# lgen-sudo/EgoM2P

Measured on AMD Instinct MI355X. Metric: multimodal tokens/sec (ego-b 400M, 10300-tok clips), training fwd+bwd+allreduce+AdamW, higher is better.
Workload: dtype bf16; 1 GPU; egom2p_base_12e_12d_swiglu_nobias mod4, synthetic 10300-position clips (1009+1009 rgb, 1009+1009 depth, 15+15 cam, 15+15 gaze kept -> N=M=2048), bf16 MFMA GEMM/attention, fp32 residual/LN/CE/AdamW; micro_batch=64, global_batch=256, parallelism=dp1

## Files before the change

egom2p_amd/_lib.py:

```python
from __future__ import annotations

import ctypes as C
import os

_HERE = os.path.dirname(os.path.abspath(__file__))
LIB_PATH = os.environ.get("EGOM2P_HIP_LIB", os.path.join(_HERE, "libegom2p_hip.so"))
MAX_MODS = 8

ABI_VERSION = 12
EPI_BF16, EPI_F32, EPI_RESID, EPI_BIAS_RESID, EPI_BIAS_BF16 = 0, 1, 2, 3, 4

vp, i32, i64, f32 = C.c_void_p, C.c_int, C.c_long, C.c_float


class CompactDesc(C.Structure):
    _fields_ = [
        ("n_mods", i32), ("n_keep", i32), ("is_decoder", i32),
        ("mask", vp * MAX_MODS), ("ids", vp * MAX_MODS), ("dam", vp * MAX_MODS),
        ("n_pos", i32 * MAX_MODS), ("mod_id", i32 * MAX_MODS),
        ("ids_keep", vp), ("pad", vp), ("mod_mask", vp), ("slot", vp), ("local", vp), ("tok", vp),
        ("ks", vp), ("ke", vp), ("n_valid", vp), ("seg", vp), ("err", vp), ("seg_bad", vp), ("n_reg", i32),
    ]


# ... 120 lines not shown
    "ego_cast_weight": [vp, i32, i32, i64, vp, i64, vp, i64, i32, vp],
    "ego_cast_f32_bf16": [vp, vp, i64, vp],
    "ego_bias_grad_work_floats": [i64, i32],
    "ego_bias_grad": [vp, i64, i32, vp, vp, i64, vp],
    "ego_grad_sqnorm": [vp, i64, vp, vp, vp],
    "ego_adamw_step": [vp, vp, vp, vp, i64, f32, f32, f32, f32, f32, i32, f32, f32, vp, i32, vp],
    "ego_adamw_gate": [vp, f32, f32, i32, vp, vp],
    "ego_adamw_step_gated": [vp, vp, vp, vp, i64, f32, f32, f32, f32, f32, i32, f32, f32, vp, i32, vp, vp],
    "ego_ema_update": [vp, vp, i64, f32, f32, vp],
    "ego_swap_f32": [vp, vp, i64, vp],
    "ego_sample_cfg_topp": [vp, vp, i64, i32, f32, f32, i32, f32, vp, vp, vp, i32, vp],
    "ego_maskgit_positions": [vp, i32, i32, i32, vp, vp],
    "ego_maskgit_select": [vp, vp, vp, i32, i32, i32, i32, vp, vp, vp, vp, vp],
    "ego_dp_unique_id": [vp],
    "ego_dp_comm_create": [vp, i32, i32, C.POINTER(vp)],
    "ego_dp_comm_destroy": [vp],
    "ego_dp_allreduce_begin": [vp, vp, i64, i32, vp, vp],
    "ego_dp_wait": [vp, vp, vp],
}

EXPORTS = tuple(_SIGS)

_SIGS_OPTIM = {
    "ego_adamw_step_seg": [vp, vp, vp, vp, i64, C.POINTER(AdamwSeg), vp, i32, vp, C.POINTER(AdamwHp), f32, f32, f32, f32, f32, vp, i32,
                           vp, vp],
}
EXPORTS_OPTIM = tuple(_SIGS_OPTIM)

OPT_ADAM, OPT_SGD, OPT_NESTEROV = 1, 2, 3
_SIGS_OPTIM_KINDS = {
    "ego_optim_step_seg": _SIGS_OPTIM["ego_adamw_step_seg"][:-1] + [i32, f32, vp],
}
EXPORTS_OPTIM_KINDS = tuple(_SIGS_OPTIM_KINDS)
_lib = None


class EgoHipError(RuntimeError):
    pass


def load():
    global _lib
    if _lib is None:
        if not os.path.exists(LIB_PATH):
            raise EgoHipError(
                f"{LIB_PATH} not found: build it with `python -c 'import __graft_entry__ as g; g.build()'` "
                "(or `make -C egom2p_amd/csrc`). There is no CPU fallback for the product path.")
        import torch
        hip_rt = os.path.join(os.path.dirname(torch.__file__), "lib", "libamdhip64.so")
        if os.path.exists(hip_rt):
            C.CDLL(hip_rt, mode=C.RTLD_GLOBAL)
        lib = C.CDLL(LIB_PATH)
        for name, args in {**_SIGS, **_SIGS_OPTIM, **_SIGS_OPTIM_KINDS}.items():
            fn = getattr(lib, name)
            fn.argtypes = args
            fn.restype = i64 if name.endswith(("_work_floats", "_split_floats", "_work_ints")) else i32
        if lib.ego_abi_version() != ABI_VERSION:
            raise EgoHipError(f"libegom2p_hip.so ABI version {lib.ego_abi_version()} != binding {ABI_VERSION}: rebuild (make -C egom2p_amd/csrc)")
        if "EGO_GEMM_NT256" in os.environ or "EGO_GEMM_TN256" in os.environ:
            lib.ego_gemm_kernel_mode(int(os.environ.get("EGO_GEMM_NT256", "1")), int(os.environ.get("EGO_GEMM_TN256", "1")))
        if "EGO_GEMM_SMALL_TILES" in os.environ:
            lib.ego_gemm_small_tiles(int(os.environ["EGO_GEMM_SMALL_TILES"]))
        _lib = lib
    return _lib


def check(rc: int, what: str):
    if rc != 0:
        raise EgoHipError(f"{what} failed: {'bad arguments' if rc == 1 else 'kernel launch failed'} (rc={rc})")
```

egom2p_amd/csrc/rowops.hip:

```cpp
#include "common.h"
#include "egom2p_hip.h"

namespace {

__device__ __forceinline__ float mul_then_add(float a, float b, float c) {
#pragma clang fp contract(off)
    const float t = a * b;
    return t + c;
}
__device__ __forceinline__ float mul_rounded(float a, float b) {
#pragma clang fp contract(off)
    return a * b;
}

constexpr int LN_MAXC_MAX = 8;

template <int LN_MAXC, bool TAIL, bool BIAS = false>
__global__ __launch_bounds__(256) void ln_fwd_kernel(const float* __restrict__ x, const float* __restrict__ w,
                                                     bf16_t* __restrict__ y, float* __restrict__ mean_out,
                                                     float* __restrict__ rstd_out, const int* __restrict__ out_row,
                                                     int rows, int D, int ld, float eps, unsigned char* __restrict__ q8, long ldq,
                                                     float* __restrict__ qscale, const float* __restrict__ b = nullptr) {
#pragma clang fp contract(off)
    const int lane = threadIdx.x & 63;
    const int row = blockIdx.x * 4 + __builtin_amdgcn_readfirstlane(threadIdx.x >> 6);
    if (row >= rows) return;
    const int nc = (D + 3) >> 2, ncl = ld >> 2;
    const float* xr = x + (long)row * ld;
    f32x4 v[LN_MAXC];
    float s = 0.f;
#pragma unroll
    for (int i = 0; i < LN_MAXC; ++i) v[i] = *(const f32x4*)(xr + min(lane + 64 * i, nc - 1) * 4);
#pragma unroll
    for (int i = 0; i < LN_MAXC; ++i) {
// ... 446 lines not shown
        const long r = idx / fc; const int c = (int)(idx % fc) * 8;
        const u32x4 a = *(const u32x4*)(u + r * ld_u + c);
        const u32x4 g = *(const u32x4*)(dh + r * ld_dh + c);
        u32x4 o;
#pragma unroll
        for (int e = 0; e < 4; ++e)
            o[e] = pack_bf16x2(bf16_to_f32(g[e] & 0xffff) * dgelu_f(bf16_to_f32(a[e] & 0xffff)),
                               bf16_to_f32(g[e] >> 16) * dgelu_f(bf16_to_f32(a[e] >> 16)));
        *(u32x4*)(du + r * ld_du + c) = o;
    }
}

__global__ __launch_bounds__(256) void cast_w_kernel(const float* __restrict__ W, int rows_src, int cols, long ld_src,
                                                     bf16_t* __restrict__ Wb, long ld_w, bf16_t* __restrict__ Wt,
                                                     long ld_t, int rows_dst) {
    __shared__ float tile[32][33];
    const int r0 = blockIdx.y * 32, c0 = blockIdx.x * 32;
    const int tx = threadIdx.x & 31, ty = threadIdx.x >> 5;
#pragma unroll
    for (int i = 0; i < 4; ++i) {
        const int r = r0 + ty + 8 * i, c = c0 + tx;
        float v = 0.f;
        if (r < rows_src && c < cols) v = W[(long)r * ld_src + c];
        tile[ty + 8 * i][tx] = v;
        if (Wb && r < rows_dst && c < cols) Wb[(long)r * ld_w + c] = f32_to_bf16(v);
    }
    __syncthreads();
    if (Wt) {
#pragma unroll
        for (int i = 0; i < 4; ++i) {
            const int c = c0 + ty + 8 * i, r = r0 + tx;
            if (c < cols && r < rows_dst) Wt[(long)c * ld_t + r] = f32_to_bf16(tile[tx][ty + 8 * i]);
        }
    }
}

__global__ __launch_bounds__(256) void ce_fwd_kernel(const bf16_t* __restrict__ logits, long ld, int V,
                                                     const int* __restrict__ targets, const int* __restrict__ range,
                                                     float* __restrict__ lse_out, float* __restrict__ nll_out) {
    __shared__ float red[8];
    const int off = range[0], n = range[1];
    const int r = blockIdx.x;
    if (r >= n) return;
    const long row = (long)off + r;
    const bf16_t* lr = logits + row * ld;
    const int lane = threadIdx.x & 63, wave = threadIdx.x >> 6;
    float mx = -3.0e38f, s = 0.f;
    const int vc = V >> 3;
    auto fold = [&](const u32x4& a) {
        float x[8];
#pragma unroll
        for (int e = 0; e < 4; ++e) { x[2 * e] = bf16_to_f32(a[e] & 0xffff); x[2 * e + 1] = bf16_to_f32(a[e] >> 16); }
        float cm = x[0];
#pragma unroll
        for (int e = 1; e < 8; ++e) cm = fmaxf(cm, x[e]);
        if (cm > mx) { s *= __expf(mx - cm); mx = cm; }
#pragma unroll
        for (int e = 0; e < 8; ++e) s += __expf(x[e] - mx);
    };
    int c = threadIdx.x;
    for (; c + 768 < vc; c += 1024) {
        const u32x4 a0 = *(const u32x4*)(lr + c * 8), a1 = *(const u32x4*)(lr + (c + 256) * 8);
        const u32x4 a2 = *(const u32x4*)(lr + (c + 512) * 8), a3 = *(const u32x4*)(lr + (c + 768) * 8);
        fold(a0); fold(a1); fold(a2); fold(a3);
    }
    for (; c < vc; c += 256) fold(*(const u32x4*)(lr + c * 8));
// ... 566 lines not shown
    if (F % 8) return EGO_ERR_ARG;
    EGO_LAUNCH(swiglu_bwd_kernel, dim3(grid_for(rows * (F / 8))), dim3(256), 0, stream, (const bf16_t*)ab, (const bf16_t*)dh, (bf16_t*)dab, rows, F);
    LAUNCH_CHECK();
    return EGO_OK;
}

extern "C" int ego_gelu_fwd(const void* u, void* h, long rows, int F, long ld_u, long ld_h, hipStream_t stream) {
    if (rows <= 0) return EGO_OK;
    if (F <= 0 || F % 8 || ld_u % 8 || ld_h % 8 || ld_u < F || ld_h < F || ((((uintptr_t)u) | ((uintptr_t)h)) & 15)) return EGO_ERR_ARG;
    EGO_LAUNCH(gelu_fwd_kernel, dim3(grid_for(rows * (F / 8))), dim3(256), 0, stream, (const bf16_t*)u, (bf16_t*)h, rows, F, ld_u, ld_h);
    LAUNCH_CHECK();
    return EGO_OK;
}

extern "C" int ego_gelu_bwd(const void* u, const void* dh, void* du, long rows, int F, long ld_u, long ld_dh, long ld_du, hipStream_t stream) {
    if (rows <= 0) return EGO_OK;
    if (F <= 0 || F % 8 || ld_u % 8 || ld_dh % 8 || ld_du % 8 || ld_u < F || ld_dh < F || ld_du < F ||
        ((((uintptr_t)u) | ((uintptr_t)dh) | ((uintptr_t)du)) & 15)) return EGO_ERR_ARG;
    EGO_LAUNCH(gelu_bwd_kernel, dim3(grid_for(rows * (F / 8))), dim3(256), 0, stream, (const bf16_t*)u, (const bf16_t*)dh, (bf16_t*)du, rows, F,
               ld_u, ld_dh, ld_du);
    LAUNCH_CHECK();
    return EGO_OK;
}

extern "C" int ego_cast_weight(const float* W, int rows, int cols, long ld_src, void* Wb, long ld_w, void* Wt, long ld_t,
                               int rows_dst, hipStream_t stream) {
    if (rows <= 0 || cols <= 0 || rows_dst < rows) return EGO_ERR_ARG;
    EGO_LAUNCH(cast_w_kernel, dim3((cols + 31) / 32, (rows_dst + 31) / 32), dim3(256), 0, stream, W, rows, cols, ld_src,
                       (bf16_t*)Wb, ld_w, (bf16_t*)Wt, ld_t, rows_dst);
    LAUNCH_CHECK();
    return EGO_OK;
}

extern "C" int ego_cast_f32_bf16(const float* src, void* dst, long n, hipStream_t stream) {
    if (n <= 0) return EGO_OK;
    if (n % 4) return EGO_ERR_ARG;
    EGO_LAUNCH(cast_f32_bf16_kernel, dim3(grid_for(n / 4)), dim3(256), 0, stream, src, (bf16_t*)dst, n / 4);
    LAUNCH_CHECK();
    return EGO_OK;
}

extern "C" int ego_ce_fwd(const void* logits, long ld, int V, const int* targets, const int* range, int max_rows,
                          float* lse, float* nll, hipStream_t stream) {
    if (max_rows <= 0) return EGO_OK;
    if (V % 8 || ld % 8) return EGO_ERR_ARG;
    EGO_LAUNCH(ce_fwd_kernel, dim3(max_rows), dim3(256), 0, stream, (const bf16_t*)logits, ld, V, targets, range, lse, nll);
    LAUNCH_CHECK();
    return EGO_OK;
}

extern "C" int ego_ce_bwd(void* logits, long ld, int V, const int* targets, const int* range, int max_rows,
                          const float* lse, const float* gscale, int n_mods, const float* loss_w, hipStream_t stream) {
    if (max_rows <= 0) return EGO_OK;
    if (V % 8 || ld % 8 || n_mods <= 0) return EGO_ERR_ARG;
    EGO_LAUNCH(ce_bwd_kernel, dim3(max_rows), dim3(256), 0, stream, (bf16_t*)logits, ld, V, targets, range, lse, gscale, 1.f / n_mods, loss_w);
    LAUNCH_CHECK();
    return EGO_OK;
}

extern "C" int ego_ce_fwd_bwd(void* logits, long ld, int V, const int* targets, const int* range, int max_rows, float* lse,
                              float* nll, const float* gscale, int n_mods, const float* loss_w, hipStream_t stream) {
    if (max_rows <= 0) return EGO_OK;
    if (V % 8 || ld % 8 || n_mods <= 0 || V > 65536) return EGO_ERR_ARG;
    if (V <= 2048) {
        EGO_LAUNCH(ce_fwd_bwd_kernel<1>, dim3(max_rows), dim3(256), 0, stream, (bf16_t*)logits, ld, V, targets, range, lse, nll, gscale, 1.f / n_mods, loss_w);
    } else {
// ... 72 lines not shown
```

egom2p_amd/engine.py:

```python
from __future__ import annotations

import math
import os
from typing import Callable, Dict, List, NamedTuple, Optional, Sequence, Tuple

import torch

from . import _lib as L
from . import ops
from .config import ModelCfg, Modality
from .posemb import build_pos_emb

BF16 = torch.bfloat16
F32 = torch.float32
I32 = torch.int32


_WARM_STREAMS: Dict[int, "torch.cuda.Stream"] = {}


def _warmup_stream(dev: torch.device) -> "torch.cuda.Stream":
    key = dev.index if dev.index is not None else torch.cuda.current_device()
    if key not in _WARM_STREAMS:
        _WARM_STREAMS[key] = torch.cuda.Stream(device=dev)
# ... 258 lines not shown
        self.n_flat_body = min([o for k, (o, _, _) in offs.items() if k.endswith("pos_emb")], default=total)
        self.P = torch.zeros(total, device=self.dev, dtype=F32)
        self.G = torch.zeros(total, device=self.dev, dtype=F32)
        self.p: Dict[str, torch.Tensor] = {}
        self.g: Dict[str, torch.Tensor] = {}
        self.offsets = offs
        for name, (o, n, shape) in offs.items():
            self.p[name] = self.P[o:o + n].view(shape)
            self.g[name] = self.G[o:o + n].view(shape)
        starts = [offs[spec[i][0]][0] for _, i in marks] + [total]
        self.buckets = [(marks[i][0], starts[i], starts[i + 1]) for i in range(len(marks))]
        self.never_grad = set() if cfg.share_embedding else {f"decoder_embeddings.{m.name}.token_emb.weight" for m in self.dec_mods}
        runs: List[List] = []
        for name, shape in spec:
            if name in self.never_grad:
                continue
            o, n, _ = offs[name]
            nd = ("norm." in name or ".norm" in name or name.endswith(".bias"))
            n4 = (n + 3) // 4 * 4
            if runs and runs[-1][2] == nd and runs[-1][1] == o:
                runs[-1][1] = o + n4
            else:
                runs.append([o, o + n4, nd])
        self.opt_runs = [(a, b, nd) for a, b, nd in runs]
        self.pos = {}
        for m in self.mods:
            pe = torch.zeros(m.max_tokens, D, device=self.dev, dtype=F32)
            pe[:, :self.Dl] = build_pos_emb(m, self.Dl)[0].to(self.dev)
            self.pos[m.name] = pe
        self.pos_enc = {m.name: self.p.get(f"encoder_embeddings.{m.name}.pos_emb", self.pos[m.name]) for m in self.enc_mods}
        self.pos_dec = {m.name: self.p.get(f"decoder_embeddings.{m.name}.pos_emb", self.pos[m.name]) for m in self.dec_mods}

        self.lin: Dict[str, _Lin] = {}

        def lin(name):
            body = "token_emb" not in name and "to_logits" not in name
            bk = name[:-len("weight")] + "bias" if name.startswith(("encoder.", "decoder.")) else None
            self.lin[name] = _Lin(name, self.p[name], self.g[name], self.dev, fp8=self.fp8_forward and body, fp8_bwd=self.fp8_backward and body,
                                  b=self.p.get(bk), gb=self.g.get(bk))

        for i in range(cfg.encoder_depth):
            for s in ("attn.qkv", "attn.proj", "mlp.fc2"):
                lin(f"encoder.{i}.{s}.weight")
            lin(f"encoder.{i}.mlp.fc1.weight") if self.gelu else self._fuse13(f"encoder.{i}")
        for i in range(cfg.decoder_depth):
            for s in ("self_attn.qkv", "self_attn.proj", "cross_attn.q", "cross_attn.kv", "cross_attn.proj", "mlp.fc2"):
                lin(f"decoder.{i}.{s}.weight")
            lin(f"decoder.{i}.mlp.fc1.weight") if self.gelu else self._fuse13(f"decoder.{i}")
        lin("decoder_proj_context.weight")
        self.logit_key = {m.name: (f"decoder_embeddings.{m.name}.token_emb.weight" if cfg.share_embedding
                                   else f"decoder_embeddings.{m.name}.to_logits.weight") for m in self.dec_mods}
        self.dec_mod_emb_key = {m.name: (f"decoder_embeddings.{m.name}.mod_emb" if m.name in self.dec_own_mod_emb
                                         else f"encoder_embeddings.{m.name}.mod_emb") for m in self.dec_mods}
        for key in self.logit_key.values():
            lin(key)

    def _fuse13(self, prefix):
        o1 = self.offsets[f"{prefix}.mlp.fc1.weight"][0]
        n = 2 * self.Fp * self.D
        w = self.P[o1:o1 + n].view(2 * self.Fp, self.D)
        g = self.G[o1:o1 + n].view(2 * self.Fp, self.D)
        self.lin[f"{prefix}.mlp.fc13"] = _Lin(f"{prefix}.mlp.fc13", w, g, self.dev, fp8=self.fp8_forward, fp8_bwd=self.fp8_backward)

    def _is_buffer_key(self, key: str) -> bool:
        return (key.endswith("pos_emb") and key not in self.p) or (not self.norm_bias and key.endswith(".bias") and "norm" in key)

# ... 126 lines not shown
            elif name.endswith("norm.weight") or ".norm" in name:
                v.fill_(1.0)
            else:
                fo, fi = self._ref_shape(name)
                if "qkv" in name: fo //= 3
                elif "kv" in name: fo //= 2
                a = math.sqrt(6.0 / (fo + fi))
                v.copy_((torch.rand(v.shape, device=self.dev, generator=gen) * 2 - 1) * a)
        bgen = torch.Generator(device=self.dev)
        bgen.manual_seed(seed + 0x5EED)
        for name in self.p:
            if name.endswith(".bias") and name != "decoder_proj_context.bias":
                v = self._view_for_key(name)
                v.copy_(torch.randn(v.shape, device=self.dev, generator=bgen) * 0.05)
        pgen = torch.Generator(device=self.dev)
        pgen.manual_seed(seed + 0x905E)
        for name in self.p:
            if name.endswith("pos_emb"):
                v = self._view_for_key(name)
                v.copy_(torch.randn(v.shape, device=self.dev, generator=pgen) * 0.02)
        self.weights_dirty = True

    def param_names(self) -> List[str]:
        return list(self.p.keys())

    def num_params(self) -> int:
        n = 0
        for name, t in self.p.items():
            v = self._view_for_key(name)
            n += v.numel()
        return n

    def refresh_weights(self):
        for name, l in self.lin.items():
            ops.cast_weight(l.w, l.wb, l.wt)
            if l.w8 is not None:
                ops.quant_fp8_rows(l.wb, l.w8, l.s8)
            if l.wt8 is not None:
                ops.quant_fp8_rows(l.wt, l.wt8, l.st8)
        self.weights_dirty = False

    def _compact_out(self, B, n_keep, train=False):
        i32 = dict(device=self.dev, dtype=I32)
        out = {k: torch.empty(B, n_keep, device=self.dev, dtype=dt) for k, dt in (
            ("ids_keep", torch.int64), ("pad", torch.uint8), ("mod_mask", torch.int16), ("slot", I32), ("local", I32), ("tok", I32),
            ("ks", I32), ("ke", I32))}
        out.update(n_valid=torch.zeros(B, **i32), seg=torch.empty(B, self.n_mods, 2, **i32), err=torch.zeros(1, **i32))
        if train:
            out["seg_bad"] = torch.zeros(B, **i32)
        return out

    def _hn_bufs(self, e, self_rows=0, q_rows=0, k_rows=0):
        if not self.qk_norm:
            return {}
        A, H = self.A, self.Hs
        out = dict(qkn=e(self_rows, 3 * A), hst=e(4, self_rows * H, dt=F32))
        if q_rows or k_rows:
            out.update(xqn=e(q_rows, A), hstq=e(2, q_rows * H, dt=F32), xkn=e(k_rows, 2 * A), hstk=e(2, k_rows * H, dt=F32))
        return out

    def _alloc_workspaces(self):
        B, N, M, D, A, Fp, H = self.Bmax, self.Ne, self.M, self.D, self.A, self.Fp, self.Hs
        dev, cfg = self.dev, self.cfg
        RN, RM = B * N, B * M

        def e(*shape, dt=BF16):
            return torch.empty(*shape, device=dev, dtype=dt)

# ... 867 lines not shown
```

egom2p_amd/ops.py:

```python
from __future__ import annotations

import ctypes as C
import os
from typing import Optional, Sequence

import torch

from . import _lib as L
from ._lib import check

BF16 = torch.bfloat16


def _p(t: Optional[torch.Tensor]):
    return None if t is None else t.data_ptr()


def _stream():
    return torch.cuda.current_stream().cuda_stream


def _need_cuda(*ts):
    for t in ts:
        if t is not None and not t.is_cuda:
# ... 281 lines not shown
    check(L.load().ego_ce_bwd(_p(logits), ld, V, _p(targets), _p(rng), max_rows, _p(lse), _p(gscale), n_mods, _p(loss_w), _stream()),
          "ego_ce_bwd")


def ce_fusable(V):
    return V % 8 == 0 and V <= 65536


def ce_fwd_bwd(logits, ld, V, targets, rng, max_rows, lse, nll, gscale, n_mods, loss_w=None):
    check(L.load().ego_ce_fwd_bwd(_p(logits), ld, V, _p(targets), _p(rng), max_rows, _p(lse), _p(nll), _p(gscale), n_mods, _p(loss_w),
                                  _stream()), "ego_ce_fwd_bwd")


LOSS_MODES = {"mod": 0, "modality": 0, "weighted_mod": 1, "token": 2}


def loss_weights(ranges, vocab, mode, loss_w, mod_scale):
    arr = (C.c_int * len(vocab))(*[int(v) for v in vocab])
    check(L.load().ego_loss_weights(_p(ranges), arr, len(vocab), mode, _p(loss_w), _p(mod_scale), _stream()), "ego_loss_weights")


def loss_finalize(nll, ranges, n_mods, out, err=None, loss_w=None, mod_scale=None):
    check(L.load().ego_loss_finalize(_p(nll), _p(ranges), n_mods, _p(out), _p(err), _p(loss_w), _p(mod_scale), _stream()),
          "ego_loss_finalize")


def cast_weight(W, Wb=None, Wt=None, rows_dst=None, ld_w=None, ld_t=None):
    rows, cols = W.shape
    rows_dst = rows if rows_dst is None else rows_dst
    ld_w = cols if ld_w is None else ld_w
    ld_t = rows_dst if ld_t is None else ld_t
    check(L.load().ego_cast_weight(_p(W), rows, cols, W.stride(0), _p(Wb), ld_w, _p(Wt), ld_t, rows_dst, _stream()),
          "ego_cast_weight")


def cast_f32_bf16(src, dst):
    check(L.load().ego_cast_f32_bf16(_p(src), _p(dst), src.numel(), _stream()), "ego_cast_f32_bf16")


def bias_grad(g, rows, D, db):
    lib = L.load()
    wk = _work(g.device, lib.ego_bias_grad_work_floats(rows, D))
    check(lib.ego_bias_grad(_p(g), rows, D, _p(db), _p(wk), wk.numel(), _stream()), "ego_bias_grad")


_SQ_WORK = {}


def grad_sqnorm(g, out):
    wk = _SQ_WORK.get(g.device)
    if wk is None:
        wk = _SQ_WORK[g.device] = torch.empty(2048, device=g.device, dtype=torch.float64)
    check(L.load().ego_grad_sqnorm(_p(g), g.numel(), _p(out), _p(wk), _stream()), "ego_grad_sqnorm")


def adamw_step(p, g, m, v, lr, wd, step, beta1=0.9, beta2=0.95, eps=1e-8, gscale=1.0, max_norm=0.0, sqnorm=None,
               zero_grad=False):
    check(L.load().ego_adamw_step(_p(p), _p(g), _p(m), _p(v), p.numel(), lr, wd, beta1, beta2, eps, step, gscale, max_norm,
                                  _p(sqnorm), int(zero_grad), _stream()), "ego_adamw_step")


GATE_WORDS = 4


def adamw_gate(sqnorm, gate, gscale=1.0, skip_norm=0.0, skip_nonfinite=False):
    if gate.dtype != torch.int32 or gate.numel() < GATE_WORDS or sqnorm.dtype != torch.float64:
# ... 251 lines not shown
```

egom2p_amd/optim.py:

```python
from __future__ import annotations

from typing import Dict, List, Optional

import torch

from . import ops


def is_no_decay(name: str, skip_list=()) -> bool:
    return "norm." in name or ".norm" in name or name.endswith(".bias") or name in skip_list


def get_num_layer_for_fm(var_name: str, num_enc_layers: int, num_dec_layers: int, last_layer_mod_emb: bool = False) -> int:
    if var_name.startswith("encoder_embeddings"):
        return 0
    if var_name.startswith("encoder."):
        return int(var_name.split(".")[1]) + 1
    if var_name in ("encoder_norm", "decoder_proj_context", "mask_token"):
        return num_enc_layers
    if not last_layer_mod_emb and var_name.startswith("decoder_embeddings.") and "mod_emb" in var_name:
        return num_enc_layers
    if var_name.startswith("decoder."):
        return num_enc_layers + int(var_name.split(".")[1]) + 1
    return num_enc_layers + num_dec_layers + 1
# ... 62 lines not shown
            launches.append((rows, list(slots)))
            rows, slots = [], {}
        if fro:
            rows.append((lo, hi, 0, 1))
        else:
            rows.append((lo, hi, slots.setdefault((grp, sk), len(slots)), 0))
    if rows:
        launches.append((rows, list(slots)))
    return launches


class FusedAdamW:

    kind = "adamw"

    def __init__(self, engine, lr: float = 1e-4, weight_decay: float = 0.05, betas=(0.9, 0.95), eps: float = 1e-8,
                 named_parameters=None, world_size: int = 1, param_groups=None):
        self.engine = engine
        self.betas, self.eps = betas, eps
        self.world_size = world_size
        self.m = torch.zeros_like(engine.P)
        self.v = torch.zeros_like(engine.P) if self.kind not in ops.SGD_KINDS else None
        self.sqnorm = torch.zeros(1, device=engine.dev, dtype=torch.float64)
        self.t = 0
        named = list(named_parameters) if named_parameters is not None else []
        self._named = named
        decay = [p for n, p in named if not is_no_decay(n)]
        nodecay = [p for n, p in named if is_no_decay(n)]
        self.param_groups: List[Dict] = [
            {"params": decay, "weight_decay": weight_decay, "lr": lr, "lr_scale": 1.0, "name": "decay"},
            {"params": nodecay, "weight_decay": 0.0, "lr": lr, "lr_scale": 1.0, "name": "no_decay"},
        ]
        self.segmented = param_groups is not None
        self._launches: List = []
        if self.segmented:
            if not named:
                raise ValueError("FusedAdamW: parameter groups need named_parameters (tensors are placed by name)")
            name_of = {id(p): n for n, p in named}
            self.param_groups, self._group_of = [], {}
            for gi, src in enumerate(param_groups):
                names = list(src.get("param_names") or [name_of[id(p)] for p in src["params"]])
                grp = {"params": list(src["params"]), "param_names": names, "weight_decay": float(src.get("weight_decay", weight_decay)),
                       "lr": float(src.get("lr", lr)), "lr_scale": float(src.get("lr_scale", 1.0)), "name": src.get("name", f"group_{gi}")}
                self.param_groups.append(grp)
                for n in names:
                    key = engine._canon_key(n)
                    if key not in engine.offsets:
                        raise ValueError(f"FusedAdamW: parameter '{n}' of group '{grp['name']}' is not a tensor of this engine")
                    if self._group_of.setdefault(key, gi) != gi:
                        raise ValueError(f"FusedAdamW: parameter '{n}' is in two groups")
            known = {engine._canon_key(n) for n, _ in named} | set(engine.never_grad)
            stray = [k for k in engine.offsets if k not in known]
            if stray:
                raise ValueError(f"FusedAdamW: engine tensors without a named parameter: {stray[:4]}")
        self._frozen_sig = None
        self._runs = [(lo, hi, nd, 0) for lo, hi, nd in engine.opt_runs]
        self._frozen_ranges: List = []
        self._frozen_names: List[str] = []
        self.skipped: Dict[str, int] = {}
        self.last_grad_norm: Optional[torch.Tensor] = None
        self.gate: Optional[torch.Tensor] = None
        self._gate_pending = False
        self._gated_base = 0

    def _fold_gated(self):
        if not self._gate_pending:
# ... 59 lines not shown
            frozen = {eng._canon_key(n) for n, p in self._named if not p.requires_grad}
            self._frozen_names = [k for k in eng.offsets if k in frozen and k in self._group_of and k not in eng.never_grad]
        return self._launches

    @torch.no_grad()
    def step(self, clip_grad: Optional[float] = None, zero_grad: bool = True, skip_grad: Optional[float] = None,
             skip_nonfinite: bool = False):
        eng = self.engine
        if getattr(eng, "params_swapped", False):
            raise RuntimeError("FusedAdamW.step inside ModelEma.applied(): the flat buffer holds the averaged weights, "
                               "a step here would train the average")
        gated = skip_grad is not None or bool(skip_nonfinite)
        if skip_grad is not None and not skip_grad > 0:
            raise ValueError(f"skip_grad must be positive, got {skip_grad}")
        self.t += 1
        gscale = 1.0 / self.world_size
        norm = None
        launches = self._plan() if self.segmented else None
        runs = self._runs if self.segmented else self._active_runs()
        if clip_grad is not None or gated:
            self.sqnorm.zero_()
            if not self._frozen_ranges:
                ops.grad_sqnorm(eng.G, self.sqnorm)
            else:
                for lo, hi, _, _ in runs:
                    ops.grad_sqnorm(eng.G[lo:hi], self.sqnorm)
            norm = self.sqnorm.sqrt().to(torch.float32) * gscale
        if gated:
            if self.gate is None:
                self.gate = torch.zeros(ops.GATE_WORDS, device=eng.dev, dtype=torch.int32)
            ops.adamw_gate(self.sqnorm, self.gate, gscale=gscale, skip_norm=float(skip_grad) if skip_grad is not None else 0.0,
                           skip_nonfinite=skip_nonfinite)
            self._gate_pending = True
        if zero_grad and not self.segmented:
            for lo, hi in self._frozen_ranges:
                eng.G[lo:hi].zero_()
        for name in self._frozen_names:
            self.skipped[name] = self.skipped.get(name, 0) + 1
        if self.segmented:
            for table, slots in launches:
                hp = [(float(self.param_groups[gi]["lr"]), float(self.param_groups[gi]["weight_decay"]), self.t - sk)
                      for gi, sk in slots] or [(0.0, 0.0, 1)]
                self._launch_seg(table, hp, gscale=gscale, max_norm=float(clip_grad) if clip_grad else 0.0,
                                 sqnorm=self.sqnorm if (clip_grad or gated) else None, zero_grad=zero_grad,
                                 gate=self.gate if gated else None)
            eng.weights_dirty = True
            self.last_grad_norm = norm
            return norm
        decay, nodecay = self.param_groups
        for lo, hi, nd, sk in runs:
            grp = nodecay if nd else decay
            if gated:
                ops.adamw_step_gated(eng.P[lo:hi], eng.G[lo:hi], self.m[lo:hi], self.v[lo:hi], float(grp["lr"]),
                                     float(grp["weight_decay"]), self.t - sk, self.gate, self.betas[0], self.betas[1], self.eps,
                                     gscale=gscale, max_norm=float(clip_grad) if clip_grad else 0.0, sqnorm=self.sqnorm,
                                     zero_grad=zero_grad)
                continue
            ops.adamw_step(eng.P[lo:hi], eng.G[lo:hi], self.m[lo:hi], self.v[lo:hi], float(grp["lr"]), float(grp["weight_decay"]),
                           self.t - sk, self.betas[0], self.betas[1], self.eps, gscale=gscale,
                           max_norm=float(clip_grad) if clip_grad else 0.0, sqnorm=self.sqnorm if clip_grad else None,
                           zero_grad=zero_grad)
        eng.weights_dirty = True
        self.last_grad_norm = norm
        return norm

    def _launch_seg(self, table, hp, **kw):
        eng = self.engine
        ops.adamw_step_seg(eng.P, eng.G, self.m, self.v, table, hp, self.betas[0], self.betas[1], self.eps, **kw)

    def zero_grad(self, set_to_none: bool = False):
        self.engine.G.zero_()

    def state_dict(self):
        self._fold_gated()
        return {"m": self.m, "v": self.v, "t": self.t, "skipped": dict(self.skipped), "layout": self.engine.layout_tag(),
                "gated_total": self.gated_total(),
                "param_groups": [{k: v for k, v in g.items() if k not in ("params", "param_names")} for g in self.param_groups]}

    def load_state_dict(self, sd):
        if sd.get("kind", "adamw") != self.kind:
            raise RuntimeError(f"optimizer state was saved by the optimiser kind '{sd.get('kind', 'adamw')}', this optimiser is "
                               f"'{self.kind}' (--opt): their state buffers mean different things; build it with the same --opt, "
                               "or restart the optimizer state")
        moments = ("m",) if self.v is None else ("m", "v")
        have, want = sd.get("layout"), self.engine.layout_tag()
        if have is None:
            raise RuntimeError("optimizer state without a storage-layout tag (saved before round 5): the flat parameter order changed since; "
                               "restart the optimizer state (the model state dict, keyed by name, still loads)")
        body = int(getattr(self.engine, "n_flat_body", want[1]))
        if (tuple(have) != tuple(want) and tuple(have[:1]) + tuple(have[2:]) == tuple(want[:1]) + tuple(want[2:])
                and int(have[1]) == body < int(want[1]) and sd["m"].numel() == body):
            for k in moments:
                getattr(self, k).zero_()
                getattr(self, k)[:body].copy_(sd[k])
            sd = dict(sd, layout=want, **{k: getattr(self, k) for k in moments},
                      skipped=dict(sd.get("skipped", {}), **{n: int(sd["t"]) for n in self.engine.offsets if n.endswith("pos_emb")}))
            have = want
# ... 134 lines not shown
```

egom2p_amd/profiler.py:

```python
from __future__ import annotations

import contextlib
from collections import defaultdict
from typing import Dict

import torch

from . import ops

PEAK_BF16_TFLOPS = 2500.0
PEAK_HBM_GBS = 8000.0


def kernel_source_sha() -> str:
    import hashlib
    import os
    root = os.path.dirname(os.path.abspath(__file__))
    files = sorted(f for f in os.listdir(os.path.join(root, "csrc")) if f.endswith((".hip", ".h")))
    h = hashlib.sha256()
    for f in files:
        h.update(f.encode())
        h.update(open(os.path.join(root, "csrc", f), "rb").read())
    return h.hexdigest()[:16]

# ... 98 lines not shown

        def c_quant(X, Q, scale, rows=None, K=None):
            r = X.shape[0] if rows is None else rows
            k = X.shape[-1] if K is None else K
            return 0.0, 3.0 * r * k

        table = {
            "gemm_nt_fp8": c_gemm_nt_fp8, "gemm_nt_swiglu_fwd_fp8": c_gemm_nt_swiglu_fwd_fp8, "quant_fp8_rows": c_quant,
            "gemm_nt": c_gemm_nt, "gemm_nt_swiglu_bwd": c_gemm_nt_swiglu_bwd, "gemm_nt_swiglu_fwd": c_gemm_nt_swiglu_fwd, "gemm_tn": c_gemm_tn, "attn_fwd": c_attn_fwd, "attn_bwd": c_attn_bwd,
            "layernorm_fwd": c_ln_fwd, "layernorm_bwd": c_ln_bwd, "layernorm_fwd_multi": c_ln_fwd_multi, "layernorm_bwd_multi": c_ln_bwd_multi, "swiglu_fwd": c_swiglu_fwd, "swiglu_bwd": c_swiglu_bwd,
            "ce_fwd": c_ce, "ce_bwd": c_ce_bwd, "ce_fwd_bwd": c_ce_bwd,
        }
        def c_compact(masks, ids, dams, n_pos, mod_ids, n_keep, is_decoder, out, B, n_reg=0, causal=False, sep=True):
            T = sum(n_pos)
            return 0.0, float(B) * (T * (1 + (4 if is_decoder else 0)) + (n_keep + n_reg) * (8 + 31))

        def c_embed_fwd(tables, pos, mod, base_vec, slot, local, tok, x, emb, rows, D, reg=None):
            n_rw = (1 if tables is not None else 0) + 1 + 1 + (1 if emb is not None else 0)
            return 0.0, float(rows) * D * 4 * n_rw + rows * 12.0

        def c_embed_bwd(dtables, dmods, dbase, dx, d2, slot, tok, rows, D, touched=None):
            n_rw = 1 + (1 if d2 is not None else 0) + (1 if dtables is not None else 0)
            return 0.0, float(rows) * D * 4 * n_rw + rows * 8.0

        def c_loss_perm(seg, canon, slot, tok, B, M, n_mods, *a):
            return 0.0, float(B) * M * 16.0

        def c_loss_finalize(nll, ranges, n_mods, out, err=None, loss_w=None, mod_scale=None):
            return 0.0, float(ranges[:n_mods, 1].sum().item()) * 4.0

        def c_cast_weight(W, Wb=None, Wt=None, **kw):
            return 0.0, float(W.numel()) * (4 + (2 if Wb is not None else 0) + (2 if Wt is not None else 0))

        def c_cast(src, dst):
            return 0.0, float(src.numel()) * 6.0

        def c_bias_grad(g, rows, D, db):
            return 0.0, float(rows) * D * 2.0

        def c_sqnorm(g, out):
            return 0.0, float(g.numel()) * 4.0

        def c_adamw(p, g, m, v, *a, zero_grad=False, **kw):
            return 0.0, float(p.numel()) * (16 + 12 + (4 if zero_grad else 0))

        def c_adamw_seg(p, g, m, v, table, hp, *a, **kw):
            return 0.0, 28.0 * table.elems_active + 4.0 * table.elems_frozen

        def c_optim_seg(kind, p, g, m, v, table, hp, *a, **kw):
            per = 20.0 if v is None else 28.0
            return 0.0, per * table.elems_active + 4.0 * table.elems_frozen

        def c_ema_update(ema, p, decay):
            return 0.0, float(ema.numel()) * 12.0

        def c_swap(a, b):
            return 0.0, float(a.numel()) * 16.0

        def c_droppath_draw(keep_prob, seed, counter, keep, B):
            return 0.0, float(keep_prob.numel()) * (4 + B)

        def c_droppath_resid(R, branch, out, keep, rows, rows_per_sample, width, keep_prob):
            return 0.0, float(rows) * width * 10.0

        def c_droppath_scale(src, dst, keep, rows, rows_per_sample, width, keep_prob):
            return 0.0, float(rows) * width * 4.0

        other = {"droppath_draw": c_droppath_draw, "droppath_resid": c_droppath_resid, "droppath_scale": c_droppath_scale,
                 "compact": c_compact, "embed_fwd": c_embed_fwd, "embed_bwd": c_embed_bwd, "loss_perm": c_loss_perm,
                 "loss_finalize": c_loss_finalize, "cast_weight": c_cast_weight, "cast_f32_bf16": c_cast, "bias_grad": c_bias_grad,
                 "grad_sqnorm": c_sqnorm, "adamw_step": c_adamw, "adamw_step_seg": c_adamw_seg, "optim_step_seg": c_optim_seg,
                 "ema_update": c_ema_update, "swap_f32": c_swap}
        self.cost_table = dict(table, **other)
        saved = {}
        family = {"gemm_nt_swiglu_fwd": "gemm_nt", "gemm_nt_swiglu_bwd": "gemm_nt"}
        for name, cost in table.items():
            saved[name] = getattr(ops, name)
            setattr(ops, name, self._wrap(family.get(name, name) if not detail_names() else name, saved[name], cost))
        for name, cost in other.items():
            saved[name] = getattr(ops, name)
            setattr(ops, name, self._wrap("other:" + name, saved[name], cost))
        try:
            yield self
        finally:
            for name, fn in saved.items():
                setattr(ops, name, fn)

    def summary(self) -> Dict[str, Dict[str, float]]:
        torch.cuda.synchronize()
        agg = defaultdict(lambda: {"ms": 0.0, "flops": 0.0, "bytes": 0.0, "calls": 0})
        for name, fl, nb, s, e in self.records:
            a = agg[name]
            a["ms"] += s.elapsed_time(e)
            a["flops"] += fl
            a["bytes"] += nb
            a["calls"] += 1
        out = {}
        for name, a in agg.items():
            sec = a["ms"] * 1e-3
            out[name] = dict(a, tflops=(a["flops"] / sec / 1e12 if sec > 0 else 0.0), gbs=(a["bytes"] / sec / 1e9 if sec > 0 else 0.0))
        return out
```

Before: 1.906 million clip-positions/s.

## Batch all weight casts into one segmented kernel and fuse AdamW runs into one launch

```diff
diff --git a/egom2p_amd/_lib.py b/egom2p_amd/_lib.py
--- a/egom2p_amd/_lib.py
+++ b/egom2p_amd/_lib.py
@@ -176,6 +176,19 @@
     "ego_optim_step_seg": _SIGS_OPTIM["ego_adamw_step_seg"][:-1] + [i32, f32, vp],
 }
 EXPORTS_OPTIM_KINDS = tuple(_SIGS_OPTIM_KINDS)
+
+CAST_TILE, CAST_VEC_SRC, CAST_VEC_WB, CAST_VEC_WT = 64, 1, 2, 4
+
+
+class CastSeg(C.Structure):
+    _fields_ = [("src", vp), ("wb", vp), ("wt", vp), ("ld_src", i64), ("ld_w", i64), ("ld_t", i64),
+                ("rows", i32), ("cols", i32), ("rows_dst", i32), ("flags", i32), ("tile0", i64)]
+
+
+_SIGS_CAST = {
+    "ego_cast_weights_seg": [C.POINTER(CastSeg), vp, i32, vp],
+}
+EXPORTS_CAST = tuple(_SIGS_CAST)
 _lib = None
 
 
@@ -195,7 +208,7 @@
         if os.path.exists(hip_rt):
             C.CDLL(hip_rt, mode=C.RTLD_GLOBAL)
         lib = C.CDLL(LIB_PATH)
-        for name, args in {**_SIGS, **_SIGS_OPTIM, **_SIGS_OPTIM_KINDS}.items():
+        for name, args in {**_SIGS, **_SIGS_OPTIM, **_SIGS_OPTIM_KINDS, **_SIGS_CAST}.items():
             fn = getattr(lib, name)
             fn.argtypes = args
             fn.restype = i64 if name.endswith(("_work_floats", "_split_floats", "_work_ints")) else i32
diff --git a/egom2p_amd/csrc/rowops.hip b/egom2p_amd/csrc/rowops.hip
--- a/egom2p_amd/csrc/rowops.hip
+++ b/egom2p_amd/csrc/rowops.hip
@@ -1,5 +1,6 @@
 #include "common.h"
 #include "egom2p_hip.h"
+#include "egom2p_hip_cast.h"
 
 namespace {
 
@@ -512,6 +513,73 @@
             const int c = c0 + ty + 8 * i, r = r0 + tx;
             if (c < cols && r < rows_dst) Wt[(long)c * ld_t + r] = f32_to_bf16(tile[tx][ty + 8 * i]);
         }
+    }
+}
+
+constexpr int CAST_T = EGO_CAST_TILE;
+static_assert(CAST_T == 64, "256 threads: 16 groups of 4 columns x 16 rows, four passes");
+
+__global__ __launch_bounds__(256) void cast_w_seg_kernel(const ego_cast_seg* __restrict__ segs, int n_segs, long n_tiles) {
+    __shared__ float tile[CAST_T][CAST_T + 1];
+    const int tx = threadIdx.x & 15, ty = threadIdx.x >> 4;
+    for (long t = blockIdx.x; t < n_tiles; t += gridDim.x) {
+        int a = 0, b = n_segs - 1;
+        while (a < b) {
+            const int mid = (a + b + 1) >> 1;
+            if (segs[mid].tile0 <= t) a = mid; else b = mid - 1;
+        }
+        const ego_cast_seg sg = segs[a];
+        const int rows = sg.rows, cols = sg.cols, rows_dst = sg.rows_dst;
+        const int tcols = (cols + CAST_T - 1) / CAST_T;
+        const long lt = t - sg.tile0;
+        if (lt < 0 || rows <= 0 || cols <= 0) continue;
+        const int r0 = (int)(lt / tcols) * CAST_T, c0 = (int)(lt % tcols) * CAST_T;
+        if (r0 >= rows_dst) continue;
+        const float* __restrict__ W = sg.src;
+        bf16_t* __restrict__ Wb = (bf16_t*)sg.wb;
+        bf16_t* __restrict__ Wt = (bf16_t*)sg.wt;
+        const bool vsrc = sg.flags & EGO_CAST_VEC_SRC, vwb = sg.flags & EGO_CAST_VEC_WB, vwt = sg.flags & EGO_CAST_VEC_WT;
+        f32x4 v[4];
+#pragma unroll
+        for (int i = 0; i < 4; ++i) {
+            const int r = r0 + ty + 16 * i, c = c0 + tx * 4;
+            v[i] = f32x4{0.f, 0.f, 0.f, 0.f};
+            if (r < rows && c < cols) {
+                if (vsrc) v[i] = *(const f32x4*)(W + (long)r * sg.ld_src + c);
+                else
+#pragma unroll
+                    for (int e = 0; e < 4; ++e) if (c + e < cols) v[i][e] = W[(long)r * sg.ld_src + c + e];
+            }
+        }
+#pragma unroll
+        for (int i = 0; i < 4; ++i) {
+            const int r = r0 + ty + 16 * i, c = c0 + tx * 4;
+#pragma unroll
+            for (int e = 0; e < 4; ++e) tile[ty + 16 * i][tx * 4 + e] = v[i][e];
+            if (Wb && r < rows_dst && c < cols) {
+                if (vwb) *(u32x2*)(Wb + (long)r * sg.ld_w + c) = u32x2{pack_bf16x2(v[i][0], v[i][1]), pack_bf16x2(v[i][2], v[i][3])};
+                else
+#pragma unroll
+                    for (int e = 0; e < 4; ++e) if (c + e < cols) Wb[(long)r * sg.ld_w + c + e] = f32_to_bf16(v[i][e]);
+            }
+        }
+        __syncthreads();
+        if (Wt) {
+#pragma unroll
+            for (int i = 0; i < 4; ++i) {
+                const int c = c0 + ty + 16 * i, r = r0 + tx * 4;
+                if (c < cols && r < rows_dst) {
+                    float o[4];
+#pragma unroll
+                    for (int e = 0; e < 4; ++e) o[e] = tile[tx * 4 + e][ty + 16 * i];
+                    if (vwt) *(u32x2*)(Wt + (long)c * sg.ld_t + r) = u32x2{pack_bf16x2(o[0], o[1]), pack_bf16x2(o[2], o[3])};
+                    else
+#pragma unroll
+                        for (int e = 0; e < 4; ++e) if (r + e < rows_dst) Wt[(long)c * sg.ld_t + r + e] = f32_to_bf16(o[e]);
+                }
+            }
+        }
+        __syncthreads();
     }
 }
 
@@ -1144,6 +1212,33 @@
     return EGO_OK;
 }
 
+namespace {
+long cast_tiles(int rows_dst, int cols) { return (long)((rows_dst + CAST_T - 1) / CAST_T) * ((cols + CAST_T - 1) / CAST_T); }
+}
+
+extern "C" int ego_cast_weights_seg(const ego_cast_seg* segs_host, const ego_cast_seg* segs, int n_segs, hipStream_t stream) {
+    if (n_segs < 0) return EGO_ERR_ARG;
+    if (n_segs == 0) return EGO_OK;
+    if (!segs_host || !segs || ((uintptr_t)segs) % 8) return EGO_ERR_ARG;
+    long n_tiles = 0;
+    for (int s = 0; s < n_segs; ++s) {
+        const ego_cast_seg& g = segs_host[s];
+        if (!g.src || g.rows <= 0 || g.cols <= 0 || g.rows_dst < g.rows || g.tile0 != n_tiles) return EGO_ERR_ARG;
+        if (g.ld_src < g.cols || (g.wb && g.ld_w < g.cols) || (g.wt && g.ld_t < g.rows_dst)) return EGO_ERR_ARG;
+        if (((uintptr_t)g.src) % 4 || ((uintptr_t)g.wb) % 2 || ((uintptr_t)g.wt) % 2) return EGO_ERR_ARG;
+        const int src_ok = g.cols % 4 == 0 && g.ld_src % 4 == 0 && ((uintptr_t)g.src) % 16 == 0;
+        const int wb_ok = g.cols % 4 == 0 && g.ld_w % 4 == 0 && ((uintptr_t)g.wb) % 8 == 0;
+        const int wt_ok = g.rows_dst % 4 == 0 && g.ld_t % 4 == 0 && ((uintptr_t)g.wt) % 8 == 0;
+        if (((g.flags & EGO_CAST_VEC_SRC) && !src_ok) || ((g.flags & EGO_CAST_VEC_WB) && !wb_ok) || ((g.flags & EGO_CAST_VEC_WT) && !wt_ok))
+            return EGO_ERR_ARG;
+        n_tiles += cast_tiles(g.rows_dst, g.cols);
+    }
+    const int blocks = (int)(n_tiles < 4096 ? n_tiles : 4096);
+    EGO_LAUNCH(cast_w_seg_kernel, dim3(blocks), dim3(256), 0, stream, segs, n_segs, n_tiles);
+    LAUNCH_CHECK();
+    return EGO_OK;
+}
+
 extern "C" int ego_cast_f32_bf16(const float* src, void* dst, long n, hipStream_t stream) {
     if (n <= 0) return EGO_OK;
     if (n % 4) return EGO_ERR_ARG;
diff --git a/egom2p_amd/engine.py b/egom2p_amd/engine.py
--- a/egom2p_amd/engine.py
+++ b/egom2p_amd/engine.py
@@ -314,6 +314,7 @@
         self.pos_dec = {m.name: self.p.get(f"decoder_embeddings.{m.name}.pos_emb", self.pos[m.name]) for m in self.dec_mods}
 
         self.lin: Dict[str, _Lin] = {}
+        self._cast_table = None
 
         def lin(name):
             body = "token_emb" not in name and "to_logits" not in name
@@ -506,8 +507,10 @@
         return n
 
     def refresh_weights(self):
+        if self._cast_table is None or len(self._cast_table) != len(self.lin):
+            self._cast_table = ops.CastSegTable([(l.w, l.wb, l.wt) for l in self.lin.values()], self.dev)
+        ops.cast_weights_seg(self._cast_table)
         for name, l in self.lin.items():
-            ops.cast_weight(l.w, l.wb, l.wt)
             if l.w8 is not None:
                 ops.quant_fp8_rows(l.wb, l.w8, l.s8)
             if l.wt8 is not None:
diff --git a/egom2p_amd/ops.py b/egom2p_amd/ops.py
--- a/egom2p_amd/ops.py
+++ b/egom2p_amd/ops.py
@@ -337,6 +337,47 @@
     ld_t = rows_dst if ld_t is None else ld_t
     check(L.load().ego_cast_weight(_p(W), rows, cols, W.stride(0), _p(Wb), ld_w, _p(Wt), ld_t, rows_dst, _stream()),
           "ego_cast_weight")
+
+
+class CastSegTable:
+
+    def __init__(self, entries, device):
+        segs, tile0, nbytes = [], 0, 0
+        self.keep = []
+        for ent in entries:
+            W, Wb, Wt = ent[:3]
+            rows_dst, ld_w, ld_t = (tuple(ent[3:]) + (None, None, None))[:3]
+            _need_cuda(W, Wb, Wt)
+            rows, cols = W.shape
+            rows_dst = rows if rows_dst is None else rows_dst
+            ld_w = cols if ld_w is None else ld_w
+            ld_t = rows_dst if ld_t is None else ld_t
+            if W.dtype != torch.float32 or W.stride(1) != 1 or any(t is not None and t.dtype != torch.bfloat16 for t in (Wb, Wt)):
+                raise L.EgoHipError("cast segment table: fp32 masters with unit column stride, bf16 copies")
+            ld_src = W.stride(0)
+            fl = 0
+            if cols % 4 == 0 and ld_src % 4 == 0 and W.data_ptr() % 16 == 0:
+                fl |= L.CAST_VEC_SRC
+            if Wb is not None and cols % 4 == 0 and ld_w % 4 == 0 and Wb.data_ptr() % 8 == 0:
+                fl |= L.CAST_VEC_WB
+            if Wt is not None and rows_dst % 4 == 0 and ld_t % 4 == 0 and Wt.data_ptr() % 8 == 0:
+                fl |= L.CAST_VEC_WT
+            segs.append(L.CastSeg(_p(W), _p(Wb), _p(Wt), ld_src, ld_w, ld_t, rows, cols, rows_dst, fl, tile0))
+            tile0 += -(-rows_dst // L.CAST_TILE) * -(-cols // L.CAST_TILE)
+            nbytes += W.numel() * (4 + (2 if Wb is not None else 0) + (2 if Wt is not None else 0))
+            self.keep.append((W, Wb, Wt))
+        self.n = len(segs)
+        self.n_tiles, self.bytes = tile0, float(nbytes)
+        self.host = (L.CastSeg * max(self.n, 1))(*segs)
+        raw = torch.frombuffer(bytearray(bytes(self.host)), dtype=torch.uint8)
+        self.dev = raw.to(device)
+
+    def __len__(self):
+        return self.n
+
+
+def cast_weights_seg(table):
+    check(L.load().ego_cast_weights_seg(table.host, _p(table.dev), len(table), _stream()), "ego_cast_weights_seg")
 
 
 def cast_f32_bf16(src, dst):
diff --git a/egom2p_amd/optim.py b/egom2p_amd/optim.py
--- a/egom2p_amd/optim.py
+++ b/egom2p_amd/optim.py
@@ -118,6 +118,8 @@
             {"params": nodecay, "weight_decay": 0.0, "lr": lr, "lr_scale": 1.0, "name": "no_decay"},
         ]
         self.segmented = param_groups is not None
+        self.one_launch = True
+        self._table_for, self._table = None, (None, None)
         self._launches: List = []
         if self.segmented:
             if not named:
@@ -243,9 +245,6 @@
             ops.adamw_gate(self.sqnorm, self.gate, gscale=gscale, skip_norm=float(skip_grad) if skip_grad is not None else 0.0,
                            skip_nonfinite=skip_nonfinite)
             self._gate_pending = True
-        if zero_grad and not self.segmented:
-            for lo, hi in self._frozen_ranges:
-                eng.G[lo:hi].zero_()
         for name in self._frozen_names:
             self.skipped[name] = self.skipped.get(name, 0) + 1
         if self.segmented:
@@ -259,6 +258,19 @@
             self.last_grad_norm = norm
             return norm
         decay, nodecay = self.param_groups
+        table, slots = self._runs_table(runs) if self.one_launch else (None, None)
+        if table is not None:
+            hp = [(float((nodecay if nd else decay)["lr"]), float((nodecay if nd else decay)["weight_decay"]), self.t - sk)
+                  for nd, sk in slots] or [(0.0, 0.0, 1)]
+            ops.adamw_step_seg(eng.P, eng.G, self.m, self.v, table, hp, self.betas[0], self.betas[1], self.eps, gscale=gscale,
+                               max_norm=float(clip_grad) if clip_grad else 0.0, sqnorm=self.sqnorm if (clip_grad or gated) else None,
+                               zero_grad=zero_grad, gate=self.gate if gated else None)
+            eng.weights_dirty = True
+            self.last_grad_norm = norm
+            return norm
+        if zero_grad:
+            for lo, hi in self._frozen_ranges:
+                eng.G[lo:hi].zero_()
         for lo, hi, nd, sk in runs:
             grp = nodecay if nd else decay
             if gated:
@@ -274,6 +286,18 @@
         eng.weights_dirty = True
         self.last_grad_norm = norm
         return norm
+
+    def _runs_table(self, runs):
+        if self._table_for is not runs:
+            rows, slots = [], {}
+            for lo, hi, nd, sk in runs:
+                rows.append((lo, hi, slots.setdefault((bool(nd), sk), len(slots)), 0))
+            rows += [(lo, hi, 0, ops.L.SEG_FROZEN) for lo, hi in self._frozen_ranges]
+            rows.sort()
+            ok = len(slots) <= ops.L.ADAMW_MAX_GROUPS
+            self._table = (ops.AdamwSegTable(rows, self.engine.dev), list(slots)) if ok else (None, None)
+            self._table_for = runs
+        return self._table
 
     def _launch_seg(self, table, hp, **kw):
         eng = self.engine
diff --git a/egom2p_amd/profiler.py b/egom2p_amd/profiler.py
--- a/egom2p_amd/profiler.py
+++ b/egom2p_amd/profiler.py
@@ -154,6 +154,9 @@
         def c_cast_weight(W, Wb=None, Wt=None, **kw):
             return 0.0, float(W.numel()) * (4 + (2 if Wb is not None else 0) + (2 if Wt is not None else 0))
 
+        def c_cast_weights_seg(table):
+            return 0.0, table.bytes
+
         def c_cast(src, dst):
             return 0.0, float(src.numel()) * 6.0
 
@@ -190,7 +193,7 @@
 
         other = {"droppath_draw": c_droppath_draw, "droppath_resid": c_droppath_resid, "droppath_scale": c_droppath_scale,
                  "compact": c_compact, "embed_fwd": c_embed_fwd, "embed_bwd": c_embed_bwd, "loss_perm": c_loss_perm,
-                 "loss_finalize": c_loss_finalize, "cast_weight": c_cast_weight, "cast_f32_bf16": c_cast, "bias_grad": c_bias_grad,
+                 "loss_finalize": c_loss_finalize, "cast_weight": c_cast_weight, "cast_weights_seg": c_cast_weights_seg, "cast_f32_bf16": c_cast, "bias_grad": c_bias_grad,
                  "grad_sqnorm": c_sqnorm, "adamw_step": c_adamw, "adamw_step_seg": c_adamw_seg, "optim_step_seg": c_optim_seg,
                  "ema_update": c_ema_update, "swap_f32": c_swap}
         self.cost_table = dict(table, **other)
diff --git a/include/egom2p_hip_cast.h b/include/egom2p_hip_cast.h
--- /dev/null
+++ b/include/egom2p_hip_cast.h
@@ -0,0 +1,30 @@
+#ifndef EGOM2P_HIP_CAST_H
+#define EGOM2P_HIP_CAST_H
+
+#include <hip/hip_runtime_api.h>
+
+#ifdef __cplusplus
+extern "C" {
+#endif
+
+#define EGO_CAST_TILE 64
+#define EGO_CAST_VEC_SRC 1
+#define EGO_CAST_VEC_WB 2
+#define EGO_CAST_VEC_WT 4
+
+typedef struct {
+    const float* src;
+    void* wb;
+    void* wt;
+    long ld_src, ld_w, ld_t;
+    int rows, cols, rows_dst, flags;
+    long tile0;
+} ego_cast_seg;
+
+int ego_cast_weights_seg(const ego_cast_seg* segs_host, const ego_cast_seg* segs, int n_segs, hipStream_t stream);
+
+#ifdef __cplusplus
+}
+#endif
+
+#endif
```

After: 1.899 million clip-positions/s. Within noise of the previous version (-0.4%).
